# yazdayy/sound-event-detection

Measured on NVIDIA B200. Metric: clips/sec (10 s, 16 kHz) logmel+CRNN inference, higher is better.
Workload: dtype fp16

## Files before the change

sound-event-detection_b200/csrc/sed_conv.cu:

```cuda
#include <cstdarg>
#include <cstdio>
#include <cstdlib>
#include <mutex>

#include "sed_conv.cuh"
#include "sed_kernels.h"

namespace sed {

static thread_local char g_err[512] = "";
const char* last_error() { return g_err; }
void set_error(const char* fmt, ...) {
  va_list ap;
  va_start(ap, fmt);
  vsnprintf(g_err, sizeof(g_err), fmt, ap);
  va_end(ap);
}

typedef CUresult (*EncodeTiledFn)(CUtensorMap*, CUtensorMapDataType, cuuint32_t, void*, const cuuint64_t*,
                                  const cuuint64_t*, const cuuint32_t*, const cuuint32_t*, CUtensorMapInterleave,
                                  CUtensorMapSwizzle, CUtensorMapL2promotion, CUtensorMapFloatOOBfill);

static EncodeTiledFn get_encode() {
  static EncodeTiledFn fn = nullptr;
// ... 257 lines not shown
  uint64_t* a_full = bars;
  uint64_t* a_empty = a_full + SA;
  uint64_t* b_full = a_empty + SA;
  uint64_t* t_full = b_full + 1;
  uint64_t* t_empty = t_full + ACC;
  uint64_t* op_full = t_empty + ACC;
  uint64_t* op_empty = op_full + 2;
  uint64_t* c1_full = op_empty + 2;
  uint64_t* c1_empty = c1_full + 2;
  uint32_t* tmem_slot = reinterpret_cast<uint32_t*>(c1_empty + 2);

  const int warp = threadIdx.x >> 5, lane = threadIdx.x & 31;
  const uint32_t rank = cluster_ctarank();
  const bool leader = rank == 0;
  const int pr_cta = blockIdx.x >> 1, npairs = gridDim.x >> 1;
  const int items = (p.num_tiles + 1) / 2;

  if (threadIdx.x < 64) {
    s_scale[threadIdx.x] = 0.25f * p.scale[threadIdx.x];
    s_shift[threadIdx.x] = 0.25f * p.shift[threadIdx.x];
    s_shift1[threadIdx.x] = p.shift1[threadIdx.x];
  }
  if (threadIdx.x >= 64 && threadIdx.x < 96) {
    const int r = threadIdx.x - 64, ch = static_cast<int>(rank) * 32 + r;
    uint32_t hi[8], lo[8];
#pragma unroll
    for (int t = 0; t < 8; ++t) {
      const float v0 = (2 * t < 9) ? p.w1[ch * 9 + 2 * t] : 0.0f;
      const float v1 = (2 * t + 1 < 9) ? p.w1[ch * 9 + 2 * t + 1] : (2 * t + 1 == 9 ? p.shift1[ch] : 0.0f);
      const __half h0 = __float2half_rn(v0), h1 = __float2half_rn(v1);
      const __half l0 = __float2half_rn(v0 - __half2float(h0)), l1 = __float2half_rn(v1 - __half2float(h1));
      hi[t] = static_cast<uint32_t>(__half_as_ushort(h0)) | (static_cast<uint32_t>(__half_as_ushort(h1)) << 16);
      lo[t] = static_cast<uint32_t>(__half_as_ushort(l0)) | (static_cast<uint32_t>(__half_as_ushort(l1)) << 16);
    }
    const int sw = (r >> 2) & 1;
    *reinterpret_cast<uint4*>(s_b1 + r * 32 + ((0 ^ sw) << 4)) = make_uint4(hi[0], hi[1], hi[2], hi[3]);
    *reinterpret_cast<uint4*>(s_b1 + r * 32 + ((1 ^ sw) << 4)) = make_uint4(hi[4], hi[0], hi[1], hi[2]);
    *reinterpret_cast<uint4*>(s_b1 + 1024 + r * 32 + ((0 ^ sw) << 4)) = make_uint4(hi[3], hi[4] & 0xFFFFu, lo[0], lo[1]);
    *reinterpret_cast<uint4*>(s_b1 + 1024 + r * 32 + ((1 ^ sw) << 4)) = make_uint4(lo[2], lo[3], lo[4], 0u);
  }
  if (warp == 0 && lane == 0) {
    tma_prefetch_desc(&tmB);
    for (int i = 0; i < SA; ++i) { mbar_init(&a_full[i], 8); mbar_init(&a_empty[i], 1); }
    mbar_init(b_full, 1);
    for (int i = 0; i < ACC; ++i) { mbar_init(&t_full[i], 1); mbar_init(&t_empty[i], 16); }
    for (int i = 0; i < 2; ++i) {
      mbar_init(&op_full[i], 8); mbar_init(&op_empty[i], 1);
      mbar_init(&c1_full[i], 1); mbar_init(&c1_empty[i], 8);
    }
    fence_barrier_init();
  }
  if (warp == 1) {
    tmem_alloc2(tmem_slot, 512);
    tmem_relinquish2();
  }
  fence_proxy_async_smem();
  tc_fence_before();
  __syncthreads();
  cluster_sync_all();
  tc_fence_after();
  const uint32_t tmem_base = *tmem_slot;

  auto tile_coords = [&](int tile, int& n, int& h0, int& w0) {
    const int per_img = p.tiles_h * p.tiles_w;
    n = fast_div(tile, p.magic_img);
    const int rem = tile - n * per_img;
    const int th = fast_div(rem, p.magic_w);
    h0 = th * 16;
    w0 = (rem - th * p.tiles_w) * 8;
  };

  if (warp < EPI_WARP0) setmaxnreg_dec<REG_CTRL>();
  if (warp >= PROD_WARP0) setmaxnreg_inc<REG_PROD>();

  if (warp == 0) {
    if (elect_one()) {
      const uint32_t bfull_leader = map_to_cta(b_full, 0);
      if (leader) mbar_expect_tx(b_full, 2 * B2_BYTES);
      for (int tap = 0; tap < 9; ++tap)
        tma_load_2d_2sm(smem_b + tap * B2_HALF, &tmB, bfull_leader, tap * 64, static_cast<int>(rank) * 32);
    }
  } else if (warp == 1) {
    if (leader && elect_one()) {
      constexpr uint32_t idesc2 = umma_idesc_f16(Elem16<T>::kFmt, 256, 64);
      constexpr uint32_t idesc1 = umma_idesc_f16(0, 256, 64);
      constexpr uint32_t a_hi = desc_hi_sw128(1280), b_hi = desc_hi_sw128(1024), d32 = desc_hi_sw32(256);
      const uint32_t a_lo0 = desc_lo(smem_u32(smem_a)), b_lo0 = desc_lo(smem_u32(smem_b));
      const uint32_t op_lo0 = desc_lo(smem_u32(s_op)), b1_hi_lo = desc_lo(smem_u32(s_b1)),
                     b1_lo_lo = desc_lo(smem_u32(s_b1 + 1024));
      mbar_wait(b_full, 0);
      tc_fence_after();
      const int n_local = (items - pr_cta + npairs - 1) / npairs;
      auto conv1 = [&](int j) {
        const int st = j & 1, ph = (j >> 1) & 1;
        mbar_wait_cluster(&op_full[st], ph);
        C1_STAMP(0, j, 0);
        mbar_wait_cluster(&c1_empty[st], ph ^ 1);
        C1_STAMP(0, j, 1);
        tc_fence_after();
        const uint32_t a_h = op_lo0 + st * (OP_STAGE >> 4), a_l = a_h + (8192 >> 4);
#pragma unroll
        for (int mt = 0; mt < 2; ++mt) {
          const uint32_t d = tmem_base + C1_COL0 + st * 128 + mt * 64;
          const uint32_t mo = mt * (4096 >> 4);
          umma_f16_2sm(d, desc_join(a_h + mo, d32), desc_join(b1_hi_lo, d32), idesc1, 0u);
          umma_f16_2sm(d, desc_join(a_l + mo, d32), desc_join(b1_lo_lo, d32), idesc1, 1u);
        }
        umma_commit_2sm(&c1_full[st], 3);
        umma_commit_2sm(&op_empty[st], 3);
      };
      uint32_t sa = 0, pa = 0, acc = 0, pacc = 0;
      if (n_local > 0) conv1(0);
      for (int i = 0; i < n_local; ++i) {
        if (i + 1 < n_local) conv1(i + 1);
        mbar_wait(&t_empty[acc], pacc ^ 1);
        C1_STAMP(0, i, 2);
        mbar_wait_cluster(&a_full[sa], pa);
        C1_STAMP(0, i, 3);
        tc_fence_after();
        const uint32_t d_base = tmem_base + acc * 64;
        const uint32_t a_lo = a_lo0 + sa * (kPatchStride >> 4);
#pragma unroll 1
        for (int tr = 0; tr < 3; ++tr) {
#pragma unroll 1
          for (int tc = 0; tc < 3; ++tc) {
            const uint32_t b_lo = b_lo0 + (tr * 3 + tc) * (B2_HALF >> 4);
            const uint32_t tap_off = (tr * 10 + tc) * 8;
#pragma unroll
            for (int k = 0; k < 4; ++k)
              umma_f16_2sm(d_base, desc_join(a_lo + tap_off + k * 2, a_hi), desc_join(b_lo + k * 2, b_hi), idesc2,
                           (tr | tc | k) ? 1u : 0u);
          }
        }
        umma_commit_2sm(&a_empty[sa], 3);
        umma_commit_2sm(&t_full[acc], 3);
        C1_STAMP(0, i, 4);
        if (++sa == SA) { sa = 0; pa ^= 1; }
        if (++acc == ACC) { acc = 0; pacc ^= 1; }
      }
    }
  } else if (warp < EPI_WARP0) {
  } else if (warp < PROD_WARP0) {
    const int quarter = warp & 3;
    const int chalf = (warp - EPI_WARP0) >> 2;
    uint32_t acc = 0, pacc = 0;
    int li = 0;
    (void)li;
    for (int w = pr_cta; w < items; w += npairs, ++li) {
      mbar_wait(&t_full[acc], pacc);
      if (warp == EPI_WARP0 && lane == 0) C1_STAMP(1, li, 0);
      tc_fence_after();
      const int tile = w * 2 + static_cast<int>(rank);
      const bool tile_ok = tile < p.num_tiles;
      int n, h0, w0;
      tile_coords(tile, n, h0, w0);
      const uint32_t taddr = tmem_base + acc * 64 + chalf * 32 + (static_cast<uint32_t>(quarter * 32) << 16);
      conv_epilogue_tile<T, 64, true, EPI_POOL>(taddr, chalf, warp, lane, s_scale, s_shift, 0, tile, tile_ok, n, h0, w0,
                                                p, nullptr, nullptr);
      tc_fence_before();
      __syncwarp();
      if (lane == 0) mbar_arrive_remote_light(&t_empty[acc], 0);
      if (warp == EPI_WARP0 && lane == 0) C1_STAMP(1, li, 1);
      if (++acc == ACC) { acc = 0; pacc ^= 1; }
    }
  } else {
    const int m_tm = (warp & 3) * 32 + lane;
    int prr[2], prc[2];
#pragma unroll
    for (int mt = 0; mt < 2; ++mt) {
      const int pr = mt * 128 + m_tm;
      prr[mt] = pr / 10;
      prc[mt] = pr - prr[mt] * 10;
    }
    const int grp = (warp - PROD_WARP0) >> 2;
    const int ptid = ((warp - PROD_WARP0) & 3) * 32 + lane;
    auto gather = [&](int tile, float (&g)[2]) {
      int n, h0, w0;
      tile_coords(tile, n, h0, w0);
      const bool tv = tile < p.num_tiles;
      const float* xn = p.x1 + static_cast<size_t>(n) * p.H * p.W;
#pragma unroll
      for (int k = 0; k < 2; ++k) {
        const int e = ptid + 128 * k;
        const int er = e / 12, ec = e - er * 12;
        const int hh = h0 - 2 + er, ww = w0 - 2 + ec;
        g[k] = (tv && e < 240 && hh >= 0 && hh < p.H && ww >= 0 && ww < p.W) ? __ldg(xn + hh * p.W + ww) : 0.0f;
      }
    };
    auto build = [&](int j, int tile, const float (&g)[2]) {
      const int st = j & 1, ph = (j >> 1) & 1;
      float* win = s_win + st * 256;
      if (ptid == 0) C1_STAMP(2, j, 0);
      win[ptid] = g[0];
      if (ptid < 112) win[128 + ptid] = g[1];
      int n, h0, w0;
      tile_coords(tile, n, h0, w0);
      const bool tv = tile < p.num_tiles;
      if (grp == 0) named_bar_sync(2, 128); else named_bar_sync(3, 128);
      if (ptid == 0) C1_STAMP(2, j, 1);
      mbar_wait(&op_empty[st], ph ^ 1);
      if (ptid == 0) C1_STAMP(2, j, 2);
      uint8_t* hi_base = s_op + st * OP_STAGE;
#pragma unroll
      for (int mt = 0; mt < 2; ++mt) {
        const int row = mt * 128 + m_tm;
        const int ph_ = h0 - 1 + prr[mt], pw_ = w0 - 1 + prc[mt];
        const bool rowv = tv && row < 180 && ph_ >= 0 && ph_ < p.H && pw_ >= 0 && pw_ < p.W;
        float in[10];
#pragma unroll
        for (int dr = 0; dr < 3; ++dr)
#pragma unroll
          for (int dc = 0; dc < 3; ++dc)
            in[dr * 3 + dc] = (rowv) ? win[(prr[mt] + dr) * 12 + prc[mt] + dc] : 0.0f;
        in[9] = rowv ? 1.0f : 0.0f;
        uint32_t hi[5], lo[5];
#pragma unroll
        for (int t = 0; t < 5; ++t) {
          const __half2 h = __floats2half2_rn(in[2 * t], in[2 * t + 1]);
          const float2 hf = __half22float2(h);
          const __half2 l = __floats2half2_rn(in[2 * t] - hf.x, in[2 * t + 1] - hf.y);
          hi[t] = *reinterpret_cast<const uint32_t*>(&h);
          lo[t] = *reinterpret_cast<const uint32_t*>(&l);
        }
        const int sw = (row >> 2) & 1;
        uint8_t* rp = hi_base + row * 32;
        *reinterpret_cast<uint4*>(rp + ((0 ^ sw) << 4)) = make_uint4(hi[0], hi[1], hi[2], hi[3]);
        *reinterpret_cast<uint4*>(rp + ((1 ^ sw) << 4)) = make_uint4(hi[4], lo[0], lo[1], lo[2]);
        *reinterpret_cast<uint4*>(rp + 8192 + ((0 ^ sw) << 4)) = make_uint4(lo[3], lo[4], hi[0], hi[1]);
        *reinterpret_cast<uint4*>(rp + 8192 + ((1 ^ sw) << 4)) = make_uint4(hi[2], hi[3], hi[4], 0u);
      }
      fence_proxy_async_smem();
      __syncwarp();
      if (lane == 0) mbar_arrive_remote_light(&op_full[st], 0);
      if (ptid == 0) C1_STAMP(2, j, 3);
    };
    auto drain = [&](int j, int tile) {
      const uint32_t sa = static_cast<uint32_t>(j) % SA, pa = (static_cast<uint32_t>(j) / SA) & 1;
      const int st = j & 1, ph = (j >> 1) & 1;
      (void)tile;
      if (ptid == 0) C1_STAMP(2, j, 4);
      mbar_wait(&c1_full[st], ph);
      if (ptid == 0) C1_STAMP(2, j, 5);
      mbar_wait(&a_empty[sa], pa ^ 1);
      if (ptid == 0) C1_STAMP(2, j, 6);
      tc_fence_after();
      uint8_t* patch = smem_a + sa * kPatchStride;
#pragma unroll
      for (int mt = 0; mt < 2; ++mt) {
        uint32_t r[4][16];
        const uint32_t taddr = tmem_base + C1_COL0 + st * 128 + mt * 64 + (static_cast<uint32_t>((warp & 3) * 32) << 16);
#pragma unroll
        for (int u = 0; u < 4; ++u) tmem_ld16(taddr + u * 16, r[u]);
        tmem_ld_wait();
        const int pr = mt * 128 + m_tm;
        if (pr < 180) {
          uint8_t* rowp = patch + pr * 128;
#pragma unroll
          for (int u = 0; u < 4; ++u) {
            uint32_t pk[8];
#pragma unroll
            for (int q = 0; q < 8; ++q)
              pk[q] = Elem16<T>::pack2_relu(__uint_as_float(r[u][2 * q]), __uint_as_float(r[u][2 * q + 1]));
            *reinterpret_cast<uint4*>(rowp + (((2 * u) ^ (pr & 7)) << 4)) = make_uint4(pk[0], pk[1], pk[2], pk[3]);
            *reinterpret_cast<uint4*>(rowp + (((2 * u + 1) ^ (pr & 7)) << 4)) = make_uint4(pk[4], pk[5], pk[6], pk[7]);
          }
        }
      }
      fence_proxy_async_smem();
      tc_fence_before();
      __syncwarp();
      if (lane == 0) {
        mbar_arrive_remote_light(&a_full[sa], 0);
        mbar_arrive_remote_light(&c1_empty[st], 0);
      }
      if (ptid == 0) C1_STAMP(2, j, 7);
    };
    float nin[2];
    auto tile_of = [&](int jj) { return (pr_cta + jj * npairs) * 2 + static_cast<int>(rank); };
    auto has = [&](int jj) { return pr_cta + jj * npairs < items; };
    int j = grp;
    if (has(j)) {
      gather(tile_of(j), nin);
      build(j, tile_of(j), nin);
      if (has(j + PG)) gather(tile_of(j + PG), nin);
    }
    for (; has(j); j += PG) {
      drain(j, tile_of(j));
      if (has(j + PG)) {
        build(j + PG, tile_of(j + PG), nin);
        if (has(j + 2 * PG)) gather(tile_of(j + 2 * PG), nin);
      }
    }
  }

  tc_fence_before();
  __syncthreads();
  cluster_sync_all();
  if (warp == 1) {
    tc_fence_after();
    tmem_dealloc2(tmem_base, 512);
  }
}


template <typename T, int CIN, int BN, int NT, bool BRES, bool PATCH, int EPI, int SA, int SB>
static int launch_cfg(const CUtensorMap& tmA, const CUtensorMap& tmB, const CUtensorMap& tmO, const ConvParams& p,
                      cudaStream_t stream) {
  using Cfg = ConvCfg<CIN, BN, NT, BRES, PATCH, EPI, SA, SB>;
  auto kern = conv_umma_kernel<T, CIN, BN, NT, BRES, PATCH, EPI, SA, SB>;
  cudaError_t e = cudaFuncSetAttribute(kern, cudaFuncAttributeMaxDynamicSharedMemorySize, Cfg::SMEM_BYTES);
  if (e != cudaSuccess) {
    set_error("cudaFuncSetAttribute(smem=%d): %s", Cfg::SMEM_BYTES, cudaGetErrorString(e));
    return SED_ERR_CUDA;
  }
  const int groups = (p.num_tiles + NT - 1) / NT;
  int grid;
  if (BRES) {
    int per_slice = num_sms() / p.nslices;
    if (per_slice > groups) per_slice = groups;
    if (per_slice < 1) per_slice = 1;
    grid = per_slice * p.nslices;
  } else {
    const long items = static_cast<long>(groups) * p.nslices;
    grid = items < num_sms() ? static_cast<int>(items) : num_sms();
  }
  kern<<<grid, Cfg::THREADS, Cfg::SMEM_BYTES, stream>>>(tmA, tmB, tmO, p);
  e = cudaGetLastError();
  if (e != cudaSuccess) {
    set_error("conv_umma launch: %s", cudaGetErrorString(e));
    return SED_ERR_CUDA;
  }
  return SED_OK;
}

template <typename T, int CIN, int BN, int EPI, int SA, int ACC, bool BRES, int NT, int SB, int EG = 1,
          bool FUSE1 = false>
static int launch_pair(const CUtensorMap& tmA, const CUtensorMap& tmB, const CUtensorMap& tmO, const ConvParams& p,
                       cudaStream_t stream) {
  using Cfg = Conv2Cfg<CIN, BN, EPI, SA, ACC, BRES, NT, SB, EG, FUSE1>;
  auto kern = conv_umma2_kernel<T, CIN, BN, EPI, SA, ACC, BRES, NT, SB, EG, FUSE1>;
  cudaError_t e = cudaFuncSetAttribute(kern, cudaFuncAttributeMaxDynamicSharedMemorySize, Cfg::SMEM_BYTES);
  if (e != cudaSuccess) {
    set_error("cudaFuncSetAttribute(pair, smem=%d): %s", Cfg::SMEM_BYTES, cudaGetErrorString(e));
    return SED_ERR_CUDA;
  }
  const int items = (p.num_tiles + 2 * NT - 1) / (2 * NT);
  int grid;
  if (BRES) {
    int pairs_per_slice = (num_sms() / 2) / p.nslices;
    if (pairs_per_slice > items) pairs_per_slice = items;
    if (pairs_per_slice < 1) pairs_per_slice = 1;
    grid = 2 * pairs_per_slice * p.nslices;
  } else {
    const long work = static_cast<long>(items) * p.nslices;
    const int pairs = num_sms() / 2;
    grid = 2 * static_cast<int>(work < pairs ? work : pairs);
  }
  kern<<<grid, Cfg::THREADS, Cfg::SMEM_BYTES, stream>>>(tmA, tmB, tmO, p);
  e = cudaGetLastError();
  if (e != cudaSuccess) {
    set_error("conv_umma2 launch: %s", cudaGetErrorString(e));
    return SED_ERR_CUDA;
  }
  return SED_OK;
}

template <typename T>
static int conv3x3_dispatch(const CUtensorMap& tmA, const CUtensorMap& tmB, const CUtensorMap& tmO, ConvParams& p,
                            int cin, int cout, int mode, int variant, cudaStream_t stream) {
  if (variant == 2) {
    if (cin == 64 && cout == 64 && mode == EPI_POOL) { p.nslices = 1; return launch_pair<T, 64, 64, EPI_POOL, 6, 4, true, 1, 1>(tmA, tmB, tmO, p, stream); }
    if (cin == 64 && cout == 128 && mode == EPI_STORE) { p.nslices = 1; return launch_pair<T, 64, 128, EPI_STORE, 4, 4, true, 1, 1>(tmA, tmB, tmO, p, stream); }
    if (cin == 128 && cout == 128 && mode == EPI_POOL) { p.nslices = 1; return launch_pair<T, 128, 128, EPI_POOL, 3, 2, true, 1, 1>(tmA, tmB, tmO, p, stream); }
    if (cin == 128 && cout == 256 && mode == EPI_STORE) { p.nslices = 2; return launch_pair<T, 128, 128, EPI_STORE, 2, 2, true, 1, 1>(tmA, tmB, tmO, p, stream); }
    if (cin == 256 && cout == 256 && mode == EPI_POOL) { p.nslices = 2; return launch_pair<T, 256, 128, EPI_POOL, 2, 2, false, 2, 6>(tmA, tmB, tmO, p, stream); }
    if (cin == 256 && cout == 512 && mode == EPI_STORE) { p.nslices = 4; return launch_pair<T, 256, 128, EPI_STORE, 2, 2, false, 2, 6>(tmA, tmB, tmO, p, stream); }
    if (cin == 512 && cout == 512 && mode == EPI_FREQMEAN) { p.nslices = 4; return launch_pair<T, 512, 128, EPI_FREQMEAN, 2, 2, false, 2, 6>(tmA, tmB, tmO, p, stream); }
    variant = 0;
  }
#define SED_CASE(CIN_, COUT_, MODE_, BN_, NT_, BRES_, SA_P, SB_P, SA_T, SB_T)                                     \
  if (cin == CIN_ && cout == COUT_ && mode == MODE_) {                                                             \
    p.nslices = COUT_ / BN_;                                                                                       \
    if (variant == 0)                                                                                              \
      return launch_cfg<T, CIN_, BN_, NT_, BRES_, true, MODE_, SA_P, SB_P>(tmA, tmB, tmO, p, stream);              \
    return launch_cfg<T, CIN_, BN_, NT_, BRES_, false, MODE_, SA_T, SB_T>(tmA, tmB, tmO, p, stream);               \
  }
  SED_CASE(64, 64, EPI_POOL, 64, 1, true, 4, 1, 6, 1)
  SED_CASE(64, 128, EPI_STORE, 128, 1, true, 2, 1, 2, 1)
  SED_CASE(128, 128, EPI_POOL, 64, 1, true, 3, 1, 4, 1)
  SED_CASE(128, 256, EPI_STORE, 64, 1, true, 2, 1, 3, 1)
  SED_CASE(256, 256, EPI_POOL, 256, 2, false, 2, 3, 3, 3)
  SED_CASE(256, 512, EPI_STORE, 256, 2, false, 2, 3, 2, 3)
  SED_CASE(512, 512, EPI_FREQMEAN, 256, 2, false, 2, 3, 3, 3)
#undef SED_CASE
  set_error("conv3x3: unsupported layer (cin=%d, cout=%d, mode=%d)", cin, cout, mode);
  return SED_ERR_UNSUPPORTED;
}

int conv3x3_launch(const void* x, int NB, int H, int W, int cin, const void* wpacked, const float* scale,
                   const float* shift, int cout, int mode, void* out, void* out_f32, long out_sn, long out_sh,
                   int dtype, int variant, cudaStream_t stream) {
  if (NB <= 0 || H <= 0 || W <= 0 || (W % 8) != 0 || (cin % 64) != 0) {
    set_error("conv3x3: bad shape NB=%d H=%d W=%d cin=%d", NB, H, W, cin);
    return SED_ERR_BAD_SHAPE;
  }
  if (mode == EPI_FREQMEAN && W != 8) {
    set_error("conv3x3: freq-mean epilogue needs W == 8 (got %d)", W);
    return SED_ERR_BAD_SHAPE;
  }
  if (mode == EPI_POOL && (W % 16) != 0) {
    set_error("conv3x3: pooling epilogue needs W %% 16 == 0 (got %d)", W);
    return SED_ERR_BAD_SHAPE;
  }
  CUtensorMap tmA, tmB;
  {
    const uint64_t dims[4] = {(uint64_t)cin, (uint64_t)W, (uint64_t)H, (uint64_t)NB};
    const uint64_t str[3] = {(uint64_t)cin * 2, (uint64_t)W * cin * 2, (uint64_t)H * W * cin * 2};
    const uint32_t box_patch[4] = {64, 10, 18, 1};
    const uint32_t box_tap[4] = {64, 8, 16, 1};
    int rc = make_map(&tmA, dtype, 4, const_cast<void*>(x), dims, str, variant != 1 ? box_patch : box_tap);
    if (rc) return rc;
  }
  int bn = 0;
  if (cin == 64 && cout == 64) bn = 64;
  else if (cin == 64 && cout == 128) bn = 128;
  else if (cin == 128) bn = 64;
  else bn = 256;
  if (variant == 2) bn = (cout == 64) ? 32 : 64;
  {
    const uint64_t dims[2] = {(uint64_t)9 * cin, (uint64_t)cout};
    const uint64_t str[1] = {(uint64_t)9 * cin * 2};
    const uint32_t box[2] = {64, (uint32_t)bn};
    int rc = make_map(&tmB, dtype, 2, const_cast<void*>(wpacked), dims, str, box);
    if (rc) return rc;
  }
  CUtensorMap tmO = tmA;
  if (mode == EPI_STORE) {
    const uint64_t dims[4] = {(uint64_t)cout, (uint64_t)W, (uint64_t)H, (uint64_t)NB};
    const uint64_t str[3] = {(uint64_t)cout * 2, (uint64_t)W * cout * 2, (uint64_t)H * W * cout * 2};
    const uint32_t box[4] = {64, 8, 16, 1};
    int rc = make_map(&tmO, dtype, 4, out, dims, str, box);
    if (rc) return rc;
  }
  ConvParams p{};
  p.NB = NB; p.H = H; p.W = W;
  p.tiles_h = (H + 15) / 16;
  p.tiles_w = W / 8;
  p.num_tiles = NB * p.tiles_h * p.tiles_w;
  {
    const unsigned long long per_img = static_cast<unsigned long long>(p.tiles_h) * p.tiles_w;
    if (per_img * (static_cast<unsigned long long>(p.num_tiles) + 4096) >= (1ull << 32)) {
      set_error("conv3x3: too many tiles for the index arithmetic (NB=%d H=%d W=%d)", NB, H, W);
      return SED_ERR_BAD_SHAPE;
    }
    p.magic_img = per_img > 1 ? static_cast<uint32_t>(((1ull << 32) + per_img - 1) / per_img) : 0u;
    p.magic_w = p.tiles_w > 1 ? static_cast<uint32_t>(((1ull << 32) + p.tiles_w - 1) / p.tiles_w) : 0u;
  }
  p.cout = cout;
  p.scale = scale; p.shift = shift;
  p.out = out; p.out2 = (mode == EPI_FREQMEAN) ? out_f32 : nullptr;
  p.M = 0; p.ldc = 0; p.relu = 1; p.tblock = 0;
  p.out_sn = (mode == EPI_FREQMEAN && out_sn > 0) ? out_sn : H;
  p.out_sh = (mode == EPI_FREQMEAN && out_sh > 0) ? out_sh : 1;
#ifdef SED_PROFILE
  {
    const char* e = getenv("SED_CONV_DBG");
    p.dbg = e ? atoi(e) : 0;
  }
#endif
  if (dtype == 0) return conv3x3_dispatch<__half>(tmA, tmB, tmO, p, cin, cout, mode, variant, stream);
  if (dtype == 1) return conv3x3_dispatch<__nv_bfloat16>(tmA, tmB, tmO, p, cin, cout, mode, variant, stream);
  set_error("conv3x3: dtype must be 0 (fp16) or 1 (bf16)");
  return SED_ERR_UNSUPPORTED;
}

int conv_block1_launch(const float* x, int NB, int H, int W, const float* w1s, const float* shift1, const void* w2packed,
                       const float* scale2, const float* shift2, void* out, int producer, int dtype,
                       cudaStream_t stream) {
  if (producer != 0 && producer != 1) {
    set_error("conv_block1: producer must be 0 (CUDA-core FMAs) or 1 (split-fp16 tensor cores)");
    return SED_ERR_UNSUPPORTED;
  }
  if (NB <= 0 || H <= 0 || W <= 0 || (W % 16) != 0) {
    set_error("conv_block1: bad shape NB=%d H=%d W=%d (W %% 16 == 0)", NB, H, W);
    return SED_ERR_BAD_SHAPE;
  }
  CUtensorMap tmB;
  {
    const uint64_t dims[2] = {(uint64_t)9 * 64, (uint64_t)64};
    const uint64_t str[1] = {(uint64_t)9 * 64 * 2};
    const uint32_t box[2] = {64, 32};
    int rc = make_map(&tmB, dtype, 2, const_cast<void*>(w2packed), dims, str, box);
    if (rc) return rc;
  }
  ConvParams p{};
  p.NB = NB; p.H = H; p.W = W;
  p.tiles_h = (H + 15) / 16;
  p.tiles_w = W / 8;
  p.num_tiles = NB * p.tiles_h * p.tiles_w;
  {
    const unsigned long long per_img = static_cast<unsigned long long>(p.tiles_h) * p.tiles_w;
    if (per_img * (static_cast<unsigned long long>(p.num_tiles) + 4096) >= (1ull << 32)) {
      set_error("conv_block1: too many tiles for the index arithmetic (NB=%d H=%d W=%d)", NB, H, W);
      return SED_ERR_BAD_SHAPE;
    }
    p.magic_img = per_img > 1 ? static_cast<uint32_t>(((1ull << 32) + per_img - 1) / per_img) : 0u;
    p.magic_w = p.tiles_w > 1 ? static_cast<uint32_t>(((1ull << 32) + p.tiles_w - 1) / p.tiles_w) : 0u;
  }
  p.cout = 64; p.nslices = 1;
  p.scale = scale2; p.shift = shift2;
  p.out = out; p.out2 = nullptr;
  p.relu = 1;
  p.out_sn = H; p.out_sh = 1;
  p.x1 = x; p.w1 = w1s; p.shift1 = shift1;
#ifdef SED_PROFILE
  {
    const char* e = getenv("SED_CONV_DBG");
    p.dbg = e ? atoi(e) : 0;
  }
#endif
  if (producer == 1) {
    if (dtype != 0 && dtype != 1) {
      set_error("conv_block1: dtype must be 0 (fp16) or 1 (bf16)");
      return SED_ERR_UNSUPPORTED;
    }
    int pairs = num_sms() / 2;
    const int items = (p.num_tiles + 1) / 2;
    if (pairs > items) pairs = items;
    cudaError_t e;
    if (dtype == 0) {
      e = cudaFuncSetAttribute(conv_block1_tc_kernel<__half>, cudaFuncAttributeMaxDynamicSharedMemorySize,
                               c1tc::SMEM_BYTES);
      if (e == cudaSuccess)
        conv_block1_tc_kernel<__half><<<2 * pairs, c1tc::THREADS, c1tc::SMEM_BYTES, stream>>>(tmB, p);
    } else {
      e = cudaFuncSetAttribute(conv_block1_tc_kernel<__nv_bfloat16>, cudaFuncAttributeMaxDynamicSharedMemorySize,
                               c1tc::SMEM_BYTES);
      if (e == cudaSuccess)
        conv_block1_tc_kernel<__nv_bfloat16><<<2 * pairs, c1tc::THREADS, c1tc::SMEM_BYTES, stream>>>(tmB, p);
    }
    if (e == cudaSuccess) e = cudaGetLastError();
    if (e != cudaSuccess) {
      set_error("conv_block1 (tensor-core producer) launch: %s", cudaGetErrorString(e));
      return SED_ERR_CUDA;
    }
    return SED_OK;
  }
  if (dtype == 0) return launch_pair<__half, 64, 64, EPI_POOL, 6, 4, true, 1, 1, 1, true>(tmB, tmB, tmB, p, stream);
  if (dtype == 1)
    return launch_pair<__nv_bfloat16, 64, 64, EPI_POOL, 6, 4, true, 1, 1, 1, true>(tmB, tmB, tmB, p, stream);
  set_error("conv_block1: dtype must be 0 (fp16) or 1 (bf16)");
  return SED_ERR_UNSUPPORTED;
}

#ifdef SED_C1_STAMPS
extern "C" int sed_debug_c1_stamps(long long* host_out) {
  return cudaMemcpyFromSymbol(host_out, g_c1_stamps, sizeof(g_c1_stamps)) == cudaSuccess ? 0 : 1;
}
#endif

int linear_launch(const void* a16, long M, int K, const void* w16, const float* bias, int N, int relu, float* out,
                  void* out16, int out_layout, int dtype, cudaStream_t stream, void* out_lo, int lo_cols) {
  if (out_lo != nullptr && (out16 == nullptr || lo_cols <= 0 || lo_cols > N || (lo_cols % 128) != 0 || N > 1536)) {
    set_error("linear: the 16-bit residual output needs the 16-bit output, lo_cols a multiple of 128 <= N <= 1536");
    return SED_ERR_BAD_SHAPE;
  }
  if (out_layout != 0 && (out_layout != 1 || out16 != nullptr || (M % 128) != 0)) {
    set_error("linear: out_layout must be 0 (row-major) or 1 (128-row transposed blocks: M %% 128 == 0, no 16-bit copy)");
    return SED_ERR_UNSUPPORTED;
  }
  if (out == nullptr && (out16 == nullptr || out_layout != 0)) {
    set_error("linear: a NULL float32 output needs the 16-bit output and the row-major layout");
    return SED_ERR_NULL;
  }
  if (M <= 0 || (N % 128) != 0 || N > 512 * 8) {
    set_error("linear: bad shape M=%ld N=%d K=%d", M, N, K);
    return SED_ERR_BAD_SHAPE;
  }
  if (K != 512 && K != 256) {
    set_error("linear: K must be 256 or 512 (got %d)", K);
    return SED_ERR_UNSUPPORTED;
  }
  CUtensorMap tmA, tmB;
  {
    const uint64_t dims[2] = {(uint64_t)K, (uint64_t)M};
    const uint64_t str[1] = {(uint64_t)K * 2};
    const uint32_t box[2] = {64, 128};
    int rc = make_map(&tmA, dtype, 2, const_cast<void*>(a16), dims, str, box);
    if (rc) return rc;
  }
  {
    const uint64_t dims[2] = {(uint64_t)K, (uint64_t)N};
    const uint64_t str[1] = {(uint64_t)K * 2};
    const uint32_t box[2] = {64, 128};
    int rc = make_map(&tmB, dtype, 2, const_cast<void*>(w16), dims, str, box);
    if (rc) return rc;
  }
  constexpr int kPanel = 1536;
  int rc = SED_OK;
  for (int n0 = 0; n0 < N && rc == SED_OK; n0 += kPanel) {
    const int npanel = (N - n0) < kPanel ? (N - n0) : kPanel;
    CUtensorMap tmBp = tmB;
    if (n0 != 0) {
      const uint64_t dims[2] = {(uint64_t)K, (uint64_t)npanel};
      const uint64_t str[1] = {(uint64_t)K * 2};
      const uint32_t box[2] = {64, 128};
      rc = make_map(&tmBp, dtype, 2, (char*)const_cast<void*>(w16) + (size_t)n0 * K * 2, dims, str, box);
      if (rc) return rc;
    }
    ConvParams p{};
    p.num_tiles = (int)((M + 127) / 128);
    p.cout = npanel;
    p.nslices = npanel / 128;
    p.scale = nullptr;
    p.shift = bias ? bias + n0 : nullptr;
    p.out = out == nullptr ? nullptr : out_layout ? out + (size_t)n0 * 128 : out + n0;
    p.out2 = out16 ? (void*)((char*)out16 + (size_t)n0 * 2) : nullptr;
    p.M = (int)M; p.ldc = N; p.relu = relu; p.tblock = out_layout;
    p.out3 = out_lo; p.lo_cols = lo_cols;
    p.out_sn = 0; p.out_sh = 0;
    if (K == 512 && M >= 128 * 296) {
      rc = dtype == 0 ? launch_cfg<__half, 512, 128, 2, false, false, EPI_LINEAR, 4, 4>(tmA, tmBp, tmA, p, stream)
                      : launch_cfg<__nv_bfloat16, 512, 128, 2, false, false, EPI_LINEAR, 4, 4>(tmA, tmBp, tmA, p, stream);
    } else if (K == 512) {
      rc = dtype == 0 ? launch_cfg<__half, 512, 128, 1, false, false, EPI_LINEAR, 4, 4>(tmA, tmBp, tmA, p, stream)
                      : launch_cfg<__nv_bfloat16, 512, 128, 1, false, false, EPI_LINEAR, 4, 4>(tmA, tmBp, tmA, p, stream);
    } else {
      rc = dtype == 0 ? launch_cfg<__half, 256, 128, 1, false, false, EPI_LINEAR, 4, 4>(tmA, tmBp, tmA, p, stream)
                      : launch_cfg<__nv_bfloat16, 256, 128, 1, false, false, EPI_LINEAR, 4, 4>(tmA, tmBp, tmA, p, stream);
    }
  }
  return rc;
}

}
```

Baseline: 49200.

## Add plane-split conv block1 kernel with 16-wide tiles and N=128 conv2 MMAs

Adds a new fused conv-block-1 kernel that stores the conv1 output patch as even and odd column planes. This lets conv2 run as wider N=128 tensor-core MMAs over 16x16 output tiles, and the 2x2 pooling is fused into the epilogue through warp shuffles. Producer mode 1 now routes to this kernel and the previous kernel moves to producer 2. The goal is fewer MMA issues per output and less epilogue work per tile, at the cost of more complex swizzled layouts and tighter shared-memory and register budgets.

Result: faster. 50380 (median of 6 runs) (+2.4%).

```diff
diff --git a/sound-event-detection_b200/csrc/sed_conv.cu b/sound-event-detection_b200/csrc/sed_conv.cu
--- a/sound-event-detection_b200/csrc/sed_conv.cu
+++ b/sound-event-detection_b200/csrc/sed_conv.cu
@@ -583,6 +583,413 @@
   }
 }
 
+namespace c1pl {
+constexpr int SA = 2;
+constexpr int ACC = 2;
+constexpr int PLANE_PX = 18 * 9;
+constexpr int PLANE = 21 * 1024;
+constexpr int A_STAGE = 2 * PLANE;
+constexpr int A_BYTES = SA * A_STAGE;
+constexpr int B2_W128 = 64 * 128, B2_W64 = 32 * 128;
+constexpr int B2_ROW = 2 * B2_W128 + 2 * B2_W64;
+constexpr int B2_BYTES = 3 * B2_ROW;
+constexpr int C1_ROWS = 384;
+constexpr int OP_LO = C1_ROWS * 32;
+constexpr int OP_STAGE = 2 * OP_LO;
+constexpr int OP_BYTES = 2 * OP_STAGE;
+constexpr int WIN = 20;
+constexpr int MISC = 3 * 256 + 2 * 2048 + 1024;
+constexpr int SMEM_BYTES = 1024 + A_BYTES + B2_BYTES + OP_BYTES + 2048 + MISC;
+static_assert(SMEM_BYTES <= 227 * 1024, "shared memory budget");
+constexpr int PG = 2;
+constexpr int EPI_WARP0 = 4, PROD_WARP0 = 12;
+constexpr int THREADS = 128 + 256 + 128 * PG;
+constexpr int REG_CTRL = 56, REG_PROD = 112;
+constexpr int C1_COL0 = ACC * 128;
+}
+
+template <typename T>
+__global__ void __cluster_dims__(2, 1, 1) __launch_bounds__(c1pl::THREADS, 1)
+conv_block1_planes_kernel(const __grid_constant__ CUtensorMap tmB, const ConvParams p) {
+  using namespace c1pl;
+  extern __shared__ uint8_t smem_raw[];
+  uint8_t* smem = align_smem_1024(smem_raw);
+  uint8_t* smem_a = smem;
+  uint8_t* smem_b = smem_a + A_BYTES;
+  uint8_t* s_op = smem_b + B2_BYTES;
+  uint8_t* s_b1 = s_op + OP_BYTES;
+  float* s_scale = reinterpret_cast<float*>(s_b1 + 2048);
+  float* s_shift = s_scale + 64;
+  float* s_shift1 = s_shift + 64;
+  float* s_win = s_shift1 + 64;
+  uint64_t* bars = reinterpret_cast<uint64_t*>(s_win + 1024);
+  uint64_t* a_full = bars;
+  uint64_t* a_empty = a_full + SA;
+  uint64_t* b_full = a_empty + SA;
+  uint64_t* t_full = b_full + 1;
+  uint64_t* t_empty = t_full + ACC;
+  uint64_t* op_full = t_empty + ACC;
+  uint64_t* op_empty = op_full + 2;
+  uint64_t* c1_full = op_empty + 2;
+  uint64_t* c1_empty = c1_full + 2;
+  uint32_t* tmem_slot = reinterpret_cast<uint32_t*>(c1_empty + 1);
+
+  const int warp = threadIdx.x >> 5, lane = threadIdx.x & 31;
+  const uint32_t rank = cluster_ctarank();
+  const bool leader = rank == 0;
+  const int pr_cta = blockIdx.x >> 1, npairs = gridDim.x >> 1;
+  const int items = (p.num_tiles + 1) / 2;
+
+  if (threadIdx.x < 64) {
+    s_scale[threadIdx.x] = 0.25f * p.scale[threadIdx.x];
+    s_shift[threadIdx.x] = 0.25f * p.shift[threadIdx.x];
+    s_shift1[threadIdx.x] = p.shift1[threadIdx.x];
+  }
+  if (threadIdx.x >= 64 && threadIdx.x < 96) {
+    const int r = threadIdx.x - 64, ch = static_cast<int>(rank) * 32 + r;
+    uint32_t hi[8], lo[8];
+#pragma unroll
+    for (int t = 0; t < 8; ++t) {
+      const float v0 = (2 * t < 9) ? p.w1[ch * 9 + 2 * t] : 0.0f;
+      const float v1 = (2 * t + 1 < 9) ? p.w1[ch * 9 + 2 * t + 1] : (2 * t + 1 == 9 ? p.shift1[ch] : 0.0f);
+      const __half h0 = __float2half_rn(v0), h1 = __float2half_rn(v1);
+      const __half l0 = __float2half_rn(v0 - __half2float(h0)), l1 = __float2half_rn(v1 - __half2float(h1));
+      hi[t] = static_cast<uint32_t>(__half_as_ushort(h0)) | (static_cast<uint32_t>(__half_as_ushort(h1)) << 16);
+      lo[t] = static_cast<uint32_t>(__half_as_ushort(l0)) | (static_cast<uint32_t>(__half_as_ushort(l1)) << 16);
+    }
+    const int sw = (r >> 2) & 1;
+    *reinterpret_cast<uint4*>(s_b1 + r * 32 + ((0 ^ sw) << 4)) = make_uint4(hi[0], hi[1], hi[2], hi[3]);
+    *reinterpret_cast<uint4*>(s_b1 + r * 32 + ((1 ^ sw) << 4)) = make_uint4(hi[4], hi[0], hi[1], hi[2]);
+    *reinterpret_cast<uint4*>(s_b1 + 1024 + r * 32 + ((0 ^ sw) << 4)) = make_uint4(hi[3], hi[4] & 0xFFFFu, lo[0], lo[1]);
+    *reinterpret_cast<uint4*>(s_b1 + 1024 + r * 32 + ((1 ^ sw) << 4)) = make_uint4(lo[2], lo[3], lo[4], 0u);
+  }
+  if (warp == 0 && lane == 0) {
+    tma_prefetch_desc(&tmB);
+    for (int i = 0; i < SA; ++i) { mbar_init(&a_full[i], 8); mbar_init(&a_empty[i], 1); }
+    mbar_init(b_full, 1);
+    for (int i = 0; i < ACC; ++i) { mbar_init(&t_full[i], 1); mbar_init(&t_empty[i], 16); }
+    for (int i = 0; i < 2; ++i) { mbar_init(&op_full[i], 8); mbar_init(&op_empty[i], 1); }
+    for (int i = 0; i < 2; ++i) mbar_init(&c1_full[i], 1);
+    mbar_init(c1_empty, 8);
+    fence_barrier_init();
+  }
+  if (warp == 1) {
+    tmem_alloc2(tmem_slot, 512);
+    tmem_relinquish2();
+  }
+  fence_proxy_async_smem();
+  tc_fence_before();
+  __syncthreads();
+  cluster_sync_all();
+  tc_fence_after();
+  const uint32_t tmem_base = *tmem_slot;
+
+  auto tile_coords = [&](int tile, int& n, int& h0, int& w0) {
+    const int per_img = p.tiles_h * p.tiles_w;
+    n = fast_div(tile, p.magic_img);
+    const int rem = tile - n * per_img;
+    const int th = fast_div(rem, p.magic_w);
+    h0 = th * 16;
+    w0 = (rem - th * p.tiles_w) * 16;
+  };
+
+  if (warp < EPI_WARP0) setmaxnreg_dec<REG_CTRL>();
+  if (warp >= PROD_WARP0) setmaxnreg_inc<REG_PROD>();
+
+  if (warp == 0) {
+    if (elect_one()) {
+      const uint32_t bfull_leader = map_to_cta(b_full, 0);
+      if (leader) mbar_expect_tx(b_full, 2 * B2_BYTES);
+      const int rk = static_cast<int>(rank);
+      for (int r = 0; r < 3; ++r) {
+        uint8_t* dst = smem_b + r * B2_ROW;
+        const int ta = r * 3 + 1 - rk, tb = r * 3 + 2 - rk;
+        for (int h = 0; h < 2; ++h) {
+          tma_load_2d_2sm(dst + h * B2_W64, &tmB, bfull_leader, ta * 64, h * 32);
+          tma_load_2d_2sm(dst + B2_W128 + h * B2_W64, &tmB, bfull_leader, tb * 64, h * 32);
+        }
+        tma_load_2d_2sm(dst + 2 * B2_W128, &tmB, bfull_leader, (r * 3) * 64, rk * 32);
+        tma_load_2d_2sm(dst + 2 * B2_W128 + B2_W64, &tmB, bfull_leader, (r * 3 + 2) * 64, rk * 32);
+      }
+    }
+  } else if (warp == 1) {
+    if (leader && elect_one()) {
+      constexpr uint32_t idesc128 = umma_idesc_f16(Elem16<T>::kFmt, 256, 128);
+      constexpr uint32_t idesc64 = umma_idesc_f16(Elem16<T>::kFmt, 256, 64);
+      constexpr uint32_t idesc1 = umma_idesc_f16(0, 256, 64);
+      constexpr uint32_t a_hi = desc_hi_sw128(9 * 128), b_hi = desc_hi_sw128(1024), d32 = desc_hi_sw32(256);
+      const uint32_t a_lo0 = desc_lo(smem_u32(smem_a)), b_lo0 = desc_lo(smem_u32(smem_b));
+      const uint32_t op_lo0 = desc_lo(smem_u32(s_op)), b1_hi_lo = desc_lo(smem_u32(s_b1)),
+                     b1_lo_lo = desc_lo(smem_u32(s_b1 + 1024));
+      mbar_wait(b_full, 0);
+      tc_fence_after();
+      const int n_local = (items - pr_cta + npairs - 1) / npairs;
+      auto conv1 = [&](int j) {
+        const int st = j & 1, ph = (j >> 1) & 1;
+        mbar_wait_cluster(&op_full[st], ph);
+        C1_STAMP(0, j, 0);
+        mbar_wait_cluster(c1_empty, (j & 1) ^ 1);
+        C1_STAMP(0, j, 1);
+        tc_fence_after();
+        const uint32_t a_h = op_lo0 + st * (OP_STAGE >> 4), a_l = a_h + (OP_LO >> 4);
+#pragma unroll
+        for (int mt = 0; mt < 3; ++mt) {
+          const uint32_t d = tmem_base + C1_COL0 + mt * 64;
+          const uint32_t mo = mt * (4096 >> 4);
+          umma_f16_2sm(d, desc_join(a_h + mo, d32), desc_join(b1_hi_lo, d32), idesc1, 0u);
+          umma_f16_2sm(d, desc_join(a_l + mo, d32), desc_join(b1_lo_lo, d32), idesc1, 1u);
+        }
+        umma_commit_2sm(&c1_full[st], 3);
+        umma_commit_2sm(&op_empty[st], 3);
+      };
+      uint32_t sa = 0, pa = 0, acc = 0, pacc = 0;
+      if (n_local > 0) conv1(0);
+      for (int i = 0; i < n_local; ++i) {
+        mbar_wait_cluster(&a_full[sa], pa);
+        C1_STAMP(0, i, 3);
+        if (i + 1 < n_local) conv1(i + 1);
+        mbar_wait(&t_empty[acc], pacc ^ 1);
+        C1_STAMP(0, i, 2);
+        tc_fence_after();
+        const uint32_t d = tmem_base + acc * 128;
+        const uint32_t e_lo = a_lo0 + sa * (A_STAGE >> 4), o_lo = e_lo + (PLANE >> 4);
+#pragma unroll 1
+        for (int r = 0; r < 3; ++r) {
+          const uint32_t e = e_lo + r * 9 * 8, o = o_lo + r * 9 * 8;
+          const uint32_t b = b_lo0 + r * (B2_ROW >> 4);
+#pragma unroll
+          for (int k = 0; k < 4; ++k)
+            umma_f16_2sm(d, desc_join(e + k * 2, a_hi), desc_join(b + k * 2, b_hi), idesc128, (r | k) ? 1u : 0u);
+#pragma unroll
+          for (int k = 0; k < 4; ++k)
+            umma_f16_2sm(d, desc_join(o + 8 + k * 2, a_hi), desc_join(b + (B2_W128 >> 4) + k * 2, b_hi), idesc128,
+                         1u);
+#pragma unroll
+          for (int k = 0; k < 4; ++k)
+            umma_f16_2sm(d, desc_join(o + k * 2, a_hi), desc_join(b + (2 * B2_W128 >> 4) + k * 2, b_hi), idesc64,
+                         1u);
+#pragma unroll
+          for (int k = 0; k < 4; ++k)
+            umma_f16_2sm(d + 64, desc_join(e + 8 + k * 2, a_hi),
+                         desc_join(b + ((2 * B2_W128 + B2_W64) >> 4) + k * 2, b_hi), idesc64, 1u);
+        }
+        umma_commit_2sm(&a_empty[sa], 3);
+        umma_commit_2sm(&t_full[acc], 3);
+        C1_STAMP(0, i, 4);
+        if (++sa == SA) { sa = 0; pa ^= 1; }
+        if (++acc == ACC) { acc = 0; pacc ^= 1; }
+      }
+    }
+  } else if (warp < EPI_WARP0) {
+  } else if (warp < PROD_WARP0) {
+    const int quarter = warp & 3;
+    const int chalf = (warp - EPI_WARP0) >> 2;
+    const int m = quarter * 32 + lane;
+    const int hl = m >> 3, jl = m & 7;
+    const bool hodd = (hl & 1) != 0;
+    const int Hp = p.H >> 1, Wp = p.W >> 1;
+    T* out16 = reinterpret_cast<T*>(p.out);
+    uint32_t acc = 0, pacc = 0;
+    int li = 0;
+    (void)li;
+    for (int w = pr_cta; w < items; w += npairs, ++li) {
+      mbar_wait(&t_full[acc], pacc);
+      if (warp == EPI_WARP0 && lane == 0) C1_STAMP(1, li, 0);
+      tc_fence_after();
+      const int tile = w * 2 + static_cast<int>(rank);
+      int n, h0, w0;
+      tile_coords(tile, n, h0, w0);
+      const int hp = (h0 + hl) >> 1, wp = (w0 >> 1) + jl;
+      const bool st_ok = tile < p.num_tiles && hp < Hp;
+      const uint32_t taddr = tmem_base + acc * 128 + (static_cast<uint32_t>(quarter * 32) << 16);
+#pragma unroll
+      for (int cb = 0; cb < 2; ++cb) {
+        const int c = chalf * 32 + cb * 16;
+        uint32_t re[16], ro[16];
+        tmem_ld16(taddr + c, re);
+        tmem_ld16(taddr + 64 + c, ro);
+        float sc[16], sh[16];
+#pragma unroll
+        for (int q = 0; q < 4; ++q) {
+          const float4 a = reinterpret_cast<const float4*>(s_scale + c)[q];
+          const float4 b = reinterpret_cast<const float4*>(s_shift + c)[q];
+          sc[4 * q] = a.x; sc[4 * q + 1] = a.y; sc[4 * q + 2] = a.z; sc[4 * q + 3] = a.w;
+          sh[4 * q] = b.x; sh[4 * q + 1] = b.y; sh[4 * q + 2] = b.z; sh[4 * q + 3] = b.w;
+        }
+        tmem_ld_wait();
+        float s[16];
+#pragma unroll
+        for (int q = 0; q < 16; ++q)
+          s[q] = fmaxf(fmaf(__uint_as_float(re[q]), sc[q], sh[q]), 0.0f) +
+                 fmaxf(fmaf(__uint_as_float(ro[q]), sc[q], sh[q]), 0.0f);
+        float k8[8];
+#pragma unroll
+        for (int q = 0; q < 8; ++q) {
+          const float send = hodd ? s[q] : s[8 + q];
+          const float keep = hodd ? s[8 + q] : s[q];
+          k8[q] = keep + __shfl_xor_sync(0xffffffffu, send, 8);
+        }
+        if (st_ok) {
+          const int ch = c + (hodd ? 8 : 0);
+          T* dst = out16 + ((static_cast<size_t>(n) * Hp + hp) * Wp + wp) * 64 + ch;
+          *reinterpret_cast<uint4*>(dst) = make_uint4(Elem16<T>::pack2(k8[0], k8[1]), Elem16<T>::pack2(k8[2], k8[3]),
+                                                      Elem16<T>::pack2(k8[4], k8[5]), Elem16<T>::pack2(k8[6], k8[7]));
+        }
+      }
+      tc_fence_before();
+      __syncwarp();
+      if (lane == 0) mbar_arrive_remote_light(&t_empty[acc], 0);
+      if (warp == EPI_WARP0 && lane == 0) C1_STAMP(1, li, 1);
+      if (++acc == ACC) { acc = 0; pacc ^= 1; }
+    }
+  } else {
+    const int m_tm = (warp & 3) * 32 + lane;
+    struct Px { int hh, cc, ofs; bool ok; };
+    auto pixel = [&](int mt) {
+      Px x;
+      const int q = mt < 2 ? mt * 128 + m_tm : 256 + (m_tm >> 5) * 17 + (m_tm & 31);
+      x.ok = mt < 2 || (m_tm & 31) < 17;
+      const int pl = q >= PLANE_PX ? 1 : 0, qq = q - pl * PLANE_PX;
+      x.hh = qq / 9;
+      x.cc = 2 * (qq - x.hh * 9) + 1 - pl;
+      x.ofs = pl * PLANE + qq * 128;
+      return x;
+    };
+    const int grp = (warp - PROD_WARP0) >> 2;
+    const int ptid = ((warp - PROD_WARP0) & 3) * 32 + lane;
+    auto gather = [&](int tile, float (&g)[4]) {
+      int n, h0, w0;
+      tile_coords(tile, n, h0, w0);
+      const bool tv = tile < p.num_tiles;
+      const float* xn = p.x1 + static_cast<size_t>(n) * p.H * p.W;
+#pragma unroll
+      for (int k = 0; k < 4; ++k) {
+        const int e = ptid + 128 * k;
+        const int er = e / WIN, ec = e - er * WIN;
+        const int hh = h0 - 2 + er, ww = w0 - 2 + ec;
+        g[k] = (tv && e < WIN * WIN && hh >= 0 && hh < p.H && ww >= 0 && ww < p.W) ? __ldg(xn + hh * p.W + ww) : 0.0f;
+      }
+    };
+    auto build = [&](int j, int tile, const float (&g)[4]) {
+      const int st = j & 1, ph = (j >> 1) & 1;
+      float* win = s_win + grp * 512;
+      if (ptid == 0) C1_STAMP(2, j, 0);
+#pragma unroll
+      for (int k = 0; k < 4; ++k)
+        if (k < 3 || ptid < WIN * WIN - 384) win[ptid + 128 * k] = g[k];
+      int n, h0, w0;
+      tile_coords(tile, n, h0, w0);
+      const bool tv = tile < p.num_tiles;
+      if (grp == 0) named_bar_sync(2, 128); else named_bar_sync(3, 128);
+      if (ptid == 0) C1_STAMP(2, j, 1);
+      mbar_wait(&op_empty[st], ph ^ 1);
+      if (ptid == 0) C1_STAMP(2, j, 2);
+      uint8_t* hi_base = s_op + st * OP_STAGE;
+#pragma unroll 1
+      for (int mt = 0; mt < 3; ++mt) {
+        const int row = mt * 128 + m_tm;
+        const Px px = pixel(mt);
+        const int ph_ = h0 - 1 + px.hh, pw_ = w0 - 1 + px.cc;
+        const bool rowv = tv && px.ok && ph_ >= 0 && ph_ < p.H && pw_ >= 0 && pw_ < p.W;
+        float in[10];
+#pragma unroll
+        for (int dr = 0; dr < 3; ++dr)
+#pragma unroll
+          for (int dc = 0; dc < 3; ++dc)
+            in[dr * 3 + dc] = (rowv) ? win[(px.hh + dr) * WIN + px.cc + dc] : 0.0f;
+        in[9] = rowv ? 1.0f : 0.0f;
+        uint32_t hi[5], lo[5];
+#pragma unroll
+        for (int t = 0; t < 5; ++t) {
+          const __half2 h = __floats2half2_rn(in[2 * t], in[2 * t + 1]);
+          const float2 hf = __half22float2(h);
+          const __half2 l = __floats2half2_rn(in[2 * t] - hf.x, in[2 * t + 1] - hf.y);
+          hi[t] = *reinterpret_cast<const uint32_t*>(&h);
+          lo[t] = *reinterpret_cast<const uint32_t*>(&l);
+        }
+        const int sw = (row >> 2) & 1;
+        uint8_t* rp = hi_base + row * 32;
+        *reinterpret_cast<uint4*>(rp + ((0 ^ sw) << 4)) = make_uint4(hi[0], hi[1], hi[2], hi[3]);
+        *reinterpret_cast<uint4*>(rp + ((1 ^ sw) << 4)) = make_uint4(hi[4], lo[0], lo[1], lo[2]);
+        *reinterpret_cast<uint4*>(rp + OP_LO + ((0 ^ sw) << 4)) = make_uint4(lo[3], lo[4], hi[0], hi[1]);
+        *reinterpret_cast<uint4*>(rp + OP_LO + ((1 ^ sw) << 4)) = make_uint4(hi[2], hi[3], hi[4], 0u);
+      }
+      fence_proxy_async_smem();
+      __syncwarp();
+      if (lane == 0) mbar_arrive_remote_light(&op_full[st], 0);
+      if (ptid == 0) C1_STAMP(2, j, 3);
+    };
+    auto drain = [&](int j) {
+      const uint32_t sa = static_cast<uint32_t>(j) % SA, pa = (static_cast<uint32_t>(j) / SA) & 1;
+      if (ptid == 0) C1_STAMP(2, j, 4);
+      mbar_wait(&c1_full[j & 1], (j >> 1) & 1);
+      if (ptid == 0) C1_STAMP(2, j, 5);
+      mbar_wait(&a_empty[sa], pa ^ 1);
+      if (ptid == 0) C1_STAMP(2, j, 6);
+      tc_fence_after();
+      uint8_t* patch = smem_a + sa * A_STAGE;
+#pragma unroll 1
+      for (int mt = 0; mt < 3; ++mt) {
+        const Px px = pixel(mt);
+        uint8_t* rowp = patch + px.ofs;
+        const int x7 = (px.ofs >> 7) & 7;
+#pragma unroll
+        for (int hf = 0; hf < 2; ++hf) {
+          uint32_t r[2][16];
+          const uint32_t taddr = tmem_base + C1_COL0 + mt * 64 + hf * 32 + (static_cast<uint32_t>((warp & 3) * 32) << 16);
+          tmem_ld16(taddr, r[0]);
+          tmem_ld16(taddr + 16, r[1]);
+          tmem_ld_wait();
+          if (px.ok) {
+#pragma unroll
+            for (int u = 0; u < 2; ++u) {
+              const int c16 = 2 * (2 * hf + u);
+              uint32_t pk[8];
+#pragma unroll
+              for (int q = 0; q < 8; ++q)
+                pk[q] = Elem16<T>::pack2_relu(__uint_as_float(r[u][2 * q]), __uint_as_float(r[u][2 * q + 1]));
+              *reinterpret_cast<uint4*>(rowp + ((c16 ^ x7) << 4)) = make_uint4(pk[0], pk[1], pk[2], pk[3]);
+              *reinterpret_cast<uint4*>(rowp + (((c16 + 1) ^ x7) << 4)) = make_uint4(pk[4], pk[5], pk[6], pk[7]);
+            }
+          }
+        }
+      }
+      fence_proxy_async_smem();
+      tc_fence_before();
+      __syncwarp();
+      if (lane == 0) {
+        mbar_arrive_remote_light(&a_full[sa], 0);
+        mbar_arrive_remote_light(c1_empty, 0);
+      }
+      if (ptid == 0) C1_STAMP(2, j, 7);
+    };
+    float nin[4];
+    auto tile_of = [&](int jj) { return (pr_cta + jj * npairs) * 2 + static_cast<int>(rank); };
+    auto has = [&](int jj) { return pr_cta + jj * npairs < items; };
+    int j = grp;
+    if (has(j)) {
+      gather(tile_of(j), nin);
+      build(j, tile_of(j), nin);
+      if (has(j + PG)) gather(tile_of(j + PG), nin);
+    }
+    for (; has(j); j += PG) {
+      drain(j);
+      if (has(j + PG)) {
+        build(j + PG, tile_of(j + PG), nin);
+        if (has(j + 2 * PG)) gather(tile_of(j + 2 * PG), nin);
+      }
+    }
+  }
+
+  tc_fence_before();
+  __syncthreads();
+  cluster_sync_all();
+  if (warp == 1) {
+    tc_fence_after();
+    tmem_dealloc2(tmem_base, 512);
+  }
+}
+
 
 template <typename T, int CIN, int BN, int NT, bool BRES, bool PATCH, int EPI, int SA, int SB>
 static int launch_cfg(const CUtensorMap& tmA, const CUtensorMap& tmB, const CUtensorMap& tmO, const ConvParams& p,
@@ -758,8 +1165,9 @@
 int conv_block1_launch(const float* x, int NB, int H, int W, const float* w1s, const float* shift1, const void* w2packed,
                        const float* scale2, const float* shift2, void* out, int producer, int dtype,
                        cudaStream_t stream) {
-  if (producer != 0 && producer != 1) {
-    set_error("conv_block1: producer must be 0 (CUDA-core FMAs) or 1 (split-fp16 tensor cores)");
+  if (producer < 0 || producer > 2) {
+    set_error("conv_block1: producer must be 0 (CUDA-core FMAs), 1 (split-fp16 tensor cores, conv2 at N = 128) or 2 "
+              "(split-fp16 tensor cores, conv2 at N = 64)");
     return SED_ERR_UNSUPPORTED;
   }
   if (NB <= 0 || H <= 0 || W <= 0 || (W % 16) != 0) {
@@ -801,6 +1209,40 @@
   }
 #endif
   if (producer == 1) {
+    if (dtype != 0 && dtype != 1) {
+      set_error("conv_block1: dtype must be 0 (fp16) or 1 (bf16)");
+      return SED_ERR_UNSUPPORTED;
+    }
+    p.tiles_w = W / 16;
+    p.num_tiles = NB * p.tiles_h * p.tiles_w;
+    {
+      const unsigned long long per_img = static_cast<unsigned long long>(p.tiles_h) * p.tiles_w;
+      p.magic_img = per_img > 1 ? static_cast<uint32_t>(((1ull << 32) + per_img - 1) / per_img) : 0u;
+      p.magic_w = p.tiles_w > 1 ? static_cast<uint32_t>(((1ull << 32) + p.tiles_w - 1) / p.tiles_w) : 0u;
+    }
+    int pairs = num_sms() / 2;
+    const int items = (p.num_tiles + 1) / 2;
+    if (pairs > items) pairs = items;
+    cudaError_t e;
+    if (dtype == 0) {
+      e = cudaFuncSetAttribute(conv_block1_planes_kernel<__half>, cudaFuncAttributeMaxDynamicSharedMemorySize,
+                               c1pl::SMEM_BYTES);
+      if (e == cudaSuccess)
+        conv_block1_planes_kernel<__half><<<2 * pairs, c1pl::THREADS, c1pl::SMEM_BYTES, stream>>>(tmB, p);
+    } else {
+      e = cudaFuncSetAttribute(conv_block1_planes_kernel<__nv_bfloat16>, cudaFuncAttributeMaxDynamicSharedMemorySize,
+                               c1pl::SMEM_BYTES);
+      if (e == cudaSuccess)
+        conv_block1_planes_kernel<__nv_bfloat16><<<2 * pairs, c1pl::THREADS, c1pl::SMEM_BYTES, stream>>>(tmB, p);
+    }
+    if (e == cudaSuccess) e = cudaGetLastError();
+    if (e != cudaSuccess) {
+      set_error("conv_block1 (tensor-core producer) launch: %s", cudaGetErrorString(e));
+      return SED_ERR_CUDA;
+    }
+    return SED_OK;
+  }
+  if (producer == 2) {
     if (dtype != 0 && dtype != 1) {
       set_error("conv_block1: dtype must be 0 (fp16) or 1 (bf16)");
       return SED_ERR_UNSUPPORTED;
```
